# dnbaker/bonsai

Hardware: AMD Instinct MI355X
Metric: reads/s classified (150 bp) (higher is better)
Workload: dtype u64

## Files before the change

bonsai_amd/csrc/bns_device.hpp:

```cpp
#pragma once
#include <hip/hip_runtime.h>
#include <stdint.h>
#include <type_traits>
#include "bns_table_plan.hpp"

namespace bns {

using u8 = uint8_t;
using u16 = uint16_t;
using u32 = uint32_t;
using u64 = uint64_t;

constexpr u32 TAX_ABSENT = 0xFFFFFFFFu;

struct alignas(16) Slot {
    u64 key;
    u32 val;
    u32 occ;
};

struct alignas(16) TaxNode {
    u32 parent;
    u32 tin, tout;
    u32 flags;
// ... 1 lines not shown
constexpr u32 NODE_PRESENT = 1u, NODE_CHAIN_OK = 2u;

__device__ __forceinline__ int lane_id() { return (int)(threadIdx.x & 63u); }

__device__ __forceinline__ u64 wang64(u64 key)
{
    key = (~key) + (key << 21);
    key = key ^ (key >> 24);
    key = (key + (key << 3)) + (key << 8);
    key = key ^ (key >> 14);
    key = (key + (key << 2)) + (key << 4);
    key = key ^ (key >> 28);
    key = key + (key << 31);
    return key;
}

__device__ __forceinline__ u32 pairswap_not(u32 x)
{
    u32 r;
    const u32 c = 0x55555555u;
    asm("v_bitop3_b32 %0, %1, %2, %3 bitop3:0x1b" : "=v"(r) : "v"(x >> 1), "v"(x << 1), "s"(c));
    return r;
}
__device__ __forceinline__ u64 revcomp(u64 kmer, u32 k)
{
    const u32 a = __builtin_bitreverse32((u32)(kmer >> 32)), b = __builtin_bitreverse32((u32)kmer);
    const u32 lo = pairswap_not(a), hi = pairswap_not(b);
    return (((u64)hi << 32) | lo) >> (64u - (k << 1));
}

__device__ __forceinline__ u64 revcomp_top(u64 win, u32 k)
{
    const u32 a = __builtin_bitreverse32((u32)(win >> 32)), b = __builtin_bitreverse32((u32)win);
    const u32 lo = pairswap_not(a), hi = pairswap_not(b);
    return (((u64)hi << 32) | lo) & (~0ULL >> (64u - (k << 1)));
}

__device__ __forceinline__ u64 revcomp64(u64 win)
{
    const u32 a = __builtin_bitreverse32((u32)(win >> 32)), b = __builtin_bitreverse32((u32)win);
    const u32 lo = pairswap_not(a), hi = pairswap_not(b);
    return ((u64)hi << 32) | lo;
}

__device__ __forceinline__ u64 canonical(u64 kmer, u32 k)
{
// ... 106 lines not shown
    u32 n;
    u32 pad;
};
static_assert(sizeof(MinBucket) == 128, "MinBucket must be one 128-byte line");
constexpr u32 MINB_N_IN_OVF = 0xFFu;
constexpr u32 MINB_HOME_SHIFT = 18u;
constexpr u32 MINB_HOME_OVF = 1u << 21;
constexpr u32 MINB_HOME_MASK = 0xFu << MINB_HOME_SHIFT;
constexpr u32 MINB_TAG_SHIFT = 22u;
constexpr u32 MINB_TAG_MASK = 0xFFu << MINB_TAG_SHIFT;
__device__ __forceinline__ u32 minb_tag(u32 minh) { return (minh * 0x85EBCA6Bu) >> 29; }
__device__ __forceinline__ u32 minb_tagbit(u32 minh) { return (1u << MINB_TAG_SHIFT) << minb_tag(minh); }
__device__ __forceinline__ u32 mph_fold(u64 key) { return (u32)key ^ __builtin_rotateleft32((u32)(key >> 32), 15); }
__device__ __forceinline__ u32 mph_slot(u32 x, u32 S) { return __umulhi(x * S, MINB_CAP); }
__device__ __forceinline__ u32 mph_candidate(u64 bucket, u32 t)
{
    u32 z = (u32)bucket * 0x9E3779B1u + t * 0x85EBCA6Bu + (u32)(bucket >> 32);
    z ^= z >> 15; z *= 0x2C1B3C6Du; z ^= z >> 12;
    return z | 1u;
}

constexpr int BNS_MAX_SPAN = 15;
__device__ __forceinline__ u32 mmer_mix(u32 h) { return h * 0x7FEB352Du; }
__device__ __forceinline__ u32 mmer_hash(u64 x)
{
    return mmer_mix((u32)x ^ __builtin_rotateleft32((u32)(x >> 32), 13));
}
__device__ __forceinline__ u64 canon_mmer(u64 fw, u32 m)
{
    const u64 r = revcomp(fw, m);
    return fw < r ? fw : r;
}
__device__ __forceinline__ u32 bucket_of(u32 minh, u32 n_mb)
{
    u32 x = minh * 0x9E3779B1u; x ^= x >> 15;
    return __umulhi(__builtin_bitreverse32(x), n_mb);
}
__device__ __forceinline__ u64 wide_ident32(u32 x) { return ((u64)__builtin_amdgcn_alignbit(0x3FFu, x * 0x7FEB352Du, 12) << 32) | x; }
__device__ __forceinline__ u64 wide_ident64(u64 x) { return 0x3FF0000000000000ULL | ((x * 0xD6E8FEB86659FD93ULL) >> 12); }
__device__ __forceinline__ u64 wide_ident(u64 x, u32 m) { return m <= 16u ? wide_ident32((u32)x) : wide_ident64(x); }
__device__ __forceinline__ u32 wide_bucket_in(u64 ident, u32 m)
{
    return m <= 16u ? (u32)ident : (u32)ident ^ (((u32)(ident >> 32) & 0xFFFFFu) * 0x85EBCA6Bu);
}
__device__ __forceinline__ u64 wide_min(u64 a, u64 b)
{
    double r;
    asm("v_min_f64 %0, %1, %2" : "=v"(r) : "v"(__builtin_bit_cast(double, a)), "v"(__builtin_bit_cast(double, b)));
    return __builtin_bit_cast(u64, r);
}
__device__ __forceinline__ u32 key_minhash(u64 key, u32 k, MinSpec sp)
{
    const u32 m = sp.m;
    const u64 mmask = ~0ULL >> (64u - 2u * m);
    if (sp.wide) {
        const u64 rc = revcomp(key, k);
        u64 best = ~0ULL;
        for (u32 i = 0; i + m <= k; ++i) {
// ... 215 lines not shown
        }
        return ProbeResult{val, (found & 1u) != 0u};
    }
    minb_ovf_walk(key, found, val, ovf_slots, ovf_mask);
    ProbeResult r{val, (found & 1u) != 0u};
    return r;
}

constexpr int MINB_NB_WIDE = 24;
template <bool KEY_MAY_BE_ONES = true, int NB = 16, bool ADJ = false>
__device__ __forceinline__ void probe_minbucket2(const MinBucket *__restrict__ buckets, u64 keyA, u32 bA, bool activeA, u64 keyB, u32 bB,
                                                 bool activeB, u32 *aux, const Slot *__restrict__ ovf_slots, u64 ovf_mask,
                                                 ProbeResult &ra, ProbeResult &rb, u32 nb = 16u)
{
    static_assert(NB == 16, "the two-key probe is built on a 16-bucket stage (two 1 KiB loads; nb = 24 adds a third)");
    const int lane = lane_id();
    u32 *list = aux;
    uint4 *stage = reinterpret_cast<uint4 *>(aux + MINB_LIST_U32);
    const uint4 *base = reinterpret_cast<const uint4 *>(buckets);
    u32 bktA = activeA ? bA : MINB_NONE, bktB = activeB ? bB : MINB_NONE;
    u32 foundA = 0u, valA = 0u, homeA = 0u, foundB = 0u, valB = 0u, homeB = 0u;
    const u32 xfA = mph_fold(keyA), xfB = mph_fold(keyB);
    constexpr u32 GO = 1u << MINB_HOME_SHIFT;
    auto look = [&](auto first_tag, u32 &bkt, u32 rank, u32 xf, u64 key, u32 &found, u32 &val, u32 home, u32 &hx) -> bool {
        constexpr bool FIRST = decltype(first_tag)::value;
        const bool mine = bkt != MINB_NONE && rank < nb;
        const char *B = reinterpret_cast<const char *>(stage) + (mine ? rank : 0u) * (16u * MINB_STRIDE);
        const uint2 hdr = *reinterpret_cast<const uint2 *>(B + 120);
        const u32 slot = mph_slot(xf, hdr.y);
        const bool eq = *reinterpret_cast<const u64 *>(B + 8u * slot) == key;
        const bool hit = mine & eq & (!KEY_MAY_BE_ONES || ((hdr.x >> (8u + slot)) & 1u));
        const u32 v = *reinterpret_cast<const u32 *>(B + 80 + 4u * slot);
        found = hit ? 1u : found;
        val = FIRST ? v : (hit ? v : val);
        bool cont;
        if (FIRST) cont = mine & !hit & ((hdr.x & (GO | 0xFFu)) >= (GO | MINB_CAP));
        else       cont = mine & !hit & ((hdr.x & 0xFFu) >= MINB_CAP) & ((((home ? home : hdr.x) & GO)) != 0u);
        bkt = (mine && !cont) ? MINB_NONE : bkt;
        hx = hdr.x;
        return cont;
    };
    auto walk = [&](auto first_tag, bool cont, u32 hx, u32 &bkt, u32 &found, u32 &home) {
        constexpr bool FIRST = decltype(first_tag)::value;
        const u32 cur = (FIRST || home == 0u) ? ((hx & MINB_HOME_MASK) | (GO << 4)) : home;
        const bool exhausted = cont && (cur >> (MINB_HOME_SHIFT + 2u)) == 0u;
        found |= (exhausted || (cont && (hx & 0xFFu) == MINB_N_IN_OVF)) ? 2u : 0u;
        const u32 next = exhausted ? MINB_NONE : bkt + 1u;
        bkt = cont ? next : bkt;
        home = cont ? cur >> 1 : home;
    };
    bool more = true;
#ifdef BNS_COUNT_FETCHES
    u32 why_later = 4u;
#endif
    auto pass = [&](auto first_tag) -> bool {
        bool pendA, chgA, pendB, chgB;
        u64 leadA, leadB;
        u32 nA;
        if constexpr (ADJ) {
            const u32 prevA = (u32)__builtin_amdgcn_update_dpp((int)~bktA, (int)bktB, DPP_WAVE_SHR1, 0xf, 0xf, false);
            pendA = bktA != MINB_NONE; chgA = bktA != prevA; pendB = bktB != MINB_NONE; chgB = bktB != bktA;
        } else {
            const u32 a63 = readlane(bktA, 63);
            const u32 prevA = (u32)__builtin_amdgcn_update_dpp((int)~bktA, (int)bktA, DPP_WAVE_SHR1, 0xf, 0xf, false);
            const u32 prevB = (u32)__builtin_amdgcn_update_dpp((int)a63, (int)bktB, DPP_WAVE_SHR1, 0xf, 0xf, false);
            pendA = bktA != MINB_NONE; chgA = bktA != prevA; pendB = bktB != MINB_NONE; chgB = bktB != prevB;
        }
        leadA = ballot64(pendA) & ballot64(chgA); leadB = ballot64(pendB) & ballot64(chgB);
        if (!(leadA | leadB)) return false;
        nA = (u32)__popcll(leadA);
        const int n_lead = (int)nA + __popcll(leadB);
#ifdef BNS_COUNT_FETCHES
        if (lane == 0) {
            atomicAdd(&g_fetch_count[0], (unsigned long long)((u32)n_lead < nb ? (u32)n_lead : nb)); atomicAdd(&g_fetch_count[1], 1ULL);
            if (!decltype(first_tag)::value) atomicAdd(&g_fetch_count[why_later], 1ULL);
        }
#endif
        u32 rankA, rankB;
        if constexpr (ADJ) {
            const u32 upA = __builtin_amdgcn_mbcnt_hi((u32)(leadA >> 33), __builtin_amdgcn_mbcnt_lo((u32)(leadA >> 1), (u32)(leadA & 1ULL) - 1u));
            rankA = __builtin_amdgcn_mbcnt_hi((u32)(leadB >> 32), __builtin_amdgcn_mbcnt_lo((u32)leadB, upA));
            rankB = rankA + ((pendB & chgB) ? 1u : 0u);
        } else {
            rankA = __builtin_amdgcn_mbcnt_hi((u32)(leadA >> 33), __builtin_amdgcn_mbcnt_lo((u32)(leadA >> 1), (u32)(leadA & 1ULL) - 1u));
            rankB = __builtin_amdgcn_mbcnt_hi((u32)(leadB >> 33), __builtin_amdgcn_mbcnt_lo((u32)(leadB >> 1), nA + (u32)(leadB & 1ULL) - 1u));
        }
        if ((pendA & chgA) && (!ADJ || rankA < nb)) list[rankA] = bktA;
        if ((pendB & chgB) && rankB < nb) list[rankB] = bktB;
        __builtin_amdgcn_wave_barrier();
        {
            const u32 last = (u32)n_lead - 1u, slot = (u32)lane >> 3;
            typedef const void __attribute__((address_space(1))) *gptr_t;
            typedef void __attribute__((address_space(3))) *lptr_t;
            const u32 b0 = list[slot < last ? slot : last];
            __builtin_amdgcn_global_load_lds((gptr_t)(base + ((u64)b0 * 8 + (u64)(lane & 7))), (lptr_t)stage, 16, 0, 2);
            if (last >= 8u) {
                const u32 b1 = list[slot + 8u < last ? slot + 8u : last];
                __builtin_amdgcn_global_load_lds((gptr_t)(base + ((u64)b1 * 8 + (u64)(lane & 7))), (lptr_t)(stage + 64), 16, 0, 2);
                if (last >= 16u && nb > 16u) {
                    const u32 b2 = list[slot + 16u < last ? slot + 16u : last];
                    __builtin_amdgcn_global_load_lds((gptr_t)(base + ((u64)b2 * 8 + (u64)(lane & 7))), (lptr_t)(stage + 128), 16, 0, 2);
                }
            }
            asm volatile("s_waitcnt vmcnt(0)" ::: "memory");
        }
        __builtin_amdgcn_wave_barrier();
        u32 hxA, hxB;
        const bool contA = look(first_tag, bktA, rankA, xfA, keyA, foundA, valA, homeA, hxA);
        const bool contB = look(first_tag, bktB, rankB, xfB, keyB, foundB, valB, homeB, hxB);
        const u64 cA = ballot64(contA), cB = ballot64(contB);
        more = (u32)n_lead > nb || (cA | cB) != 0ULL;
#ifdef BNS_COUNT_FETCHES
        why_later = 4u + ((u32)n_lead > nb ? 1u : 0u) + ((cA | cB) != 0ULL ? 2u : 0u);
#endif
        if (cA) walk(first_tag, contA, hxA, bktA, foundA, homeA);
        if (cB) walk(first_tag, contB, hxB, bktB, foundB, homeB);
        __builtin_amdgcn_wave_barrier();
        return true;
    };
    if (pass(std::true_type{}) && more) {
        while (more && pass(std::false_type{})) {}
#ifdef BNS_COUNT_FETCHES
        { const u64 gA = ballot64(foundA == 2u), gB = ballot64(foundB == 2u);
          if ((gA | gB) && lane == 0) { atomicAdd(&g_fetch_count[2], (unsigned long long)(__popcll(gA) + __popcll(gB))); atomicAdd(&g_fetch_count[3], 1ULL); } }
#endif
        minb_ovf_walk(keyA, foundA, valA, ovf_slots, ovf_mask);
        minb_ovf_walk(keyB, foundB, valB, ovf_slots, ovf_mask);
    }
    ra = ProbeResult{valA, foundA == 1u};
    rb = ProbeResult{valB, foundB == 1u};
}

__device__ __forceinline__ TaxNode load_node(const TaxNode *__restrict__ nodes, u32 n_nodes, u32 id)
{
    if (id < n_nodes) return nodes[id];
    return TaxNode{TAX_ABSENT, 0u, 0u, 0u};
}

__device__ __forceinline__ bool anc_or_self(u32 x, const TaxNode &nx, u32 a, const TaxNode &na)
{
    return x == a || (nx.tin < na.tin && na.tin < nx.tout);
}

__device__ inline u32 lca_dev(const TaxNode *__restrict__ nodes, u32 n_nodes, u32 a, u32 b)
{
    if (a == b) return a;
    if (b == 0) return a;
    if (a == 0) return b;
// ... 13 lines not shown
```

bonsai_amd/csrc/bns_kernels.hip:

```cpp
#include "bns_device.hpp"
#include "bns_kernels.hpp"

namespace bns {

typedef const volatile __attribute__((address_space(4))) ClassifyParams ColdParams;
__device__ __forceinline__ ColdParams *cold_params() { return (ColdParams *)__builtin_amdgcn_kernarg_segment_ptr(); }

__device__ __forceinline__ u32 base_code(u32 b, u32 &bad)
{
    const u32 c = b & 0xDFu;
    const bool ok = (c == 0x41u) | (c == 0x43u) | (c == 0x47u) | (c == 0x54u);
    const u32 x = (c >> 1) & 3u;
    bad = ok ? 0u : 1u;
    return ok ? (x ^ (x >> 1)) : 0u;
}

__global__ __launch_bounds__(256) void pack_kernel(const u8 *__restrict__ bases, const u64 *__restrict__ offsets,
                                                   u64 n_reads, u64 *__restrict__ words, u32 *__restrict__ nmask)
{
    const int lane = lane_id();
    const u64 wave = (u64)blockIdx.x * (blockDim.x >> 6) + (u64)__builtin_amdgcn_readfirstlane((int)(threadIdx.x >> 6));
    const u64 n_waves = (u64)gridDim.x * (blockDim.x >> 6);
    for (u64 r = wave; r < n_reads; r += n_waves) {
        const u64 o = offsets[r];
// ... 36 lines not shown
        }
    }
}

template <bool ZEROED = false>
__device__ __forceinline__ void raw_load(const u8 *__restrict__ bases, u64 o, u32 L, u32 first_base, u32 &lo, u32 &hi)
{
    const u32 bi = first_base + (u32)lane_id() * 4u;
    if (!ZEROED) { lo = 0; hi = 0; }
    if (bi < L) {
        const u64 addr = o + bi;
        const u32 mis = (u32)(addr & 3u);
        const u32 *ap = reinterpret_cast<const u32 *>(bases + (addr - mis));
        const u32 nbytes = (L - bi) < 4u ? (L - bi) : 4u;
        lo = ap[0];
        if (mis + nbytes > 4u) hi = ap[1];
    }
}

__device__ __forceinline__ void swar_codes2(u32 w, u32 nvalid, u32 &codes8, u32 &mask8, u32 &bad8)
{
    const u32 x = w & 0xDFDFDFDFu;
    const u32 sel = (x >> 1) & 0x03030303u;
    const u32 expect = __builtin_amdgcn_perm(0u, 0x47544341u, sel);
    const u32 diff = expect ^ x;
    const u32 nz = (((diff & 0x7F7F7F7Fu) + 0x7F7F7F7Fu) | diff) & 0x80808080u;
    const u32 inv3 = (nz >> 7) * 3u;
    const u32 c = (sel ^ ((sel >> 1) & 0x01010101u)) & ~inv3;
    const u32 tail = 0xFFu >> (2u * nvalid);
    codes8 = ((c * 0x40100401u) >> 24) & ~tail;
    const u32 inv8 = (inv3 * 0x40100401u) >> 24;
    mask8 = inv8 | tail;
    bad8 = inv8 & ~tail;
}

constexpr u32 IMG_N32 = 130;
constexpr u32 IMG_U64 = 130;
template <bool ORD32 = false>
__device__ __forceinline__ bool pack_chunk_lds(const u8 *__restrict__ bases, u64 offv, int mate, u32 L, u32 j0, bool have0, u32 r_lo, u32 r_hi, u64 *pk)
{
    const int lane = lane_id();
    const u32 rem = L - j0;
    const u32 n_pass = rem >= 2048u ? 8u : (rem + 255u) >> 8;
    const u32 mis8 = 8u * ((readlane((u32)offv, mate) + j0) & 3u);
    u8 *pc = reinterpret_cast<u8 *>(pk) + (ORD32 ? 4 : 0), *pm = ORD32 ? reinterpret_cast<u8 *>(pk) + 4u * IMG_N32 + 4 : reinterpret_cast<u8 *>(pk + 64);
    u64 dirty = 0;
    auto convert = [&](u32 pass, u32 lo, u32 hi) {
        const u32 w = (u32)((((u64)hi << 32) | lo) >> mis8);
        const u32 bi = j0 + pass * 256u + (u32)lane * 4u;
        u32 codes, mask, bad;
        swar_codes2(w, bi < L ? (L - bi < 4u ? L - bi : 4u) : 0u, codes, mask, bad);
        dirty |= ballot64(bad != 0u);
        const u32 at = pass * 64u + ((u32)lane ^ (ORD32 ? 3u : 7u));
        pc[at] = (u8)codes;
        pm[at] = (u8)mask;
    };
    if (n_pass) {
        u32 lo = r_lo, hi = r_hi;
        if (!have0) { raw_load(bases, readlane64(offv, mate), L, j0, lo, hi); asm volatile("" : "+v"(lo), "+v"(hi)); }
        convert(0u, lo, hi);
    }
    for (u32 pass = 1; pass < n_pass; ++pass) {
        u32 lo, hi;
        raw_load(bases, readlane64(offv, mate), L, j0 + pass * 256u, lo, hi);
        convert(pass, lo, hi);
    }
    __builtin_amdgcn_wave_barrier();
    return dirty == 0;
}

struct Prefetch { u32 lo, hi, m; };
template <bool PACKED>
__device__ __forceinline__ void prefetch_clear(Prefetch &f)
{
// ... 169 lines not shown
__device__ __forceinline__ void window16_min2(u32 h0, u32 h1, u32 g0, u32 g1, u32 *ring, u32 &wA, u32 &wB)
{
    const u32 lane = (u32)lane_id();
    uint2 *ring2 = reinterpret_cast<uint2 *>(ring);
    const u32 Xv = blk8_suffix_min(min(g0, g1));
    ring2[lane] = make_uint2(Xv, min(Xv, dpp<0x111>(g1)));
    __builtin_amdgcn_wave_barrier();
    const u32 pm = min(h0, h1);
    const u32 P = blk8_prefix_min(pm), S = blk8_suffix_min(pm);
    ring2[8u + lane] = make_uint2(min(h1, blk8_exclusive(S, false)), S);
    __builtin_amdgcn_wave_barrier();
    const u32 xin = ring[2u * lane], sin = ring[2u * lane + 3u];
    __builtin_amdgcn_wave_barrier();
    wA = min(min(xin, blk8_exclusive(P, true)), h0);
    wB = min(sin, P);
}

template <int SPAN>
__device__ __forceinline__ void round2_minhash(u64 kfA, u64 rcA, u64 kfB, u64 rcB, u32 m, u32 *ring, u32 &hA, u32 &hB)
{
    static_assert(SPAN >= 2, "a window of at least three m-mers");
    const u32 lane = (u32)lane_id();
    const u64 mmask = ~0ULL >> (64u - 2u * m);
    auto canon_hash = [&](u64 a, u64 b) -> u32 {
        if (m <= 16u) return mmer_mix(min((u32)a, (u32)b));
        return mmer_hash(a < b ? a : b);
    };
    const u32 g0 = canon_hash(kfA >> (2u * SPAN), rcA & mmask), g1 = canon_hash(kfB >> (2u * SPAN), rcB & mmask);
    const u32 h0 = canon_hash(kfA & mmask, rcA >> (2u * SPAN)), h1 = canon_hash(kfB & mmask, rcB >> (2u * SPAN));
    if (SPAN == 15) { window16_min2(h0, h1, g0, g1, ring, hA, hB); return; }
    u32 c = min(g1, h0);
    constexpr u32 NP = ((u32)SPAN - 1u) / 2u;
    if (NP) {
        uint2 *ring2 = reinterpret_cast<uint2 *>(ring);
        ring2[lane] = make_uint2(g0, g1);
        ring[2u * lane + (u32)SPAN] = h0; ring[2u * lane + (u32)SPAN + 1u] = h1;
        __builtin_amdgcn_wave_barrier();
        uint2 h[NP ? NP : 1u];
#pragma unroll
        for (u32 i = 0; i < NP; ++i) h[i] = ring2[lane + 1u + i];
#pragma unroll
        for (u32 i = 0; i < NP; ++i) c = min(min(c, h[i].x), h[i].y);
        __builtin_amdgcn_wave_barrier();
    }
    hA = min(c, g0);
    hB = min(c, h1);
}

template <int W, bool VH = false>
__device__ __forceinline__ u32 round_minhash(u64 kf, u64 rc, u32 rd, u32 k, u32 m, u32 *ring, u32 lane_ = (u32)lane_id())
{
    const int lane = (int)lane_;
    const u32 span = k - m;
    const u64 mmask = ~0ULL >> (64u - 2u * m);
    if (span == 0) { const u64 a = kf & mmask, b = rc & mmask; return mmer_hash(a < b ? a : b); }
    u32 mine;
    if (VH) {
        u32 head = 0;
        if (m <= 16u) {
            const u32 mm = 0xFFFFFFFFu >> (32u - 2u * m);
            if (rd == 0) head = mmer_mix(min((u32)(kf >> 30) & mm, (u32)rc & mm));
            mine = mmer_mix(min((u32)kf & mm, (u32)(rc >> 30)));
        } else {
            if (rd == 0) { const u64 a = kf >> 30, b = rc & mmask; head = mmer_hash(a < b ? a : b); }
            const u64 a = kf & mmask, b = rc >> 30;
            mine = mmer_hash(a < b ? a : b);
        }
        return window16_min(mine, head, rd, ring, lane_);
    }
    if (m <= 16u) {
        const u32 mm = 0xFFFFFFFFu >> (32u - 2u * m);
        if (rd == 0) { asm volatile(""); if ((u32)lane < span) ring[lane] = mmer_mix(min((u32)(kf >> (2u * span)) & mm, (u32)rc & mm)); }
        mine = mmer_mix(min((u32)kf & mm, (u32)(rc >> (2u * span))));
        ring[span + (u32)lane] = mine;
    } else {
        if (rd == 0) {
            if ((u32)lane < span) {
                const u64 a = kf >> (2u * span), b = rc & mmask;
                ring[lane] = mmer_hash(a < b ? a : b);
            }
        }
        const u64 a = kf & mmask, b = rc >> (2u * span);
        mine = mmer_hash(a < b ? a : b);
        ring[span + (u32)lane] = mine;
    }
    __builtin_amdgcn_wave_barrier();
    constexpr u32 G = W <= 9 ? (u32)W : ((u32)W + 1u) / 2u;
    u32 best = 0xFFFFFFFFu;
#pragma unroll
    for (u32 g = 0; g < (u32)W; g += G) {
        u32 h[G + 1];
#pragma unroll
        for (u32 i = 0; i <= G; ++i) h[i] = (i < G && g + i < (u32)W) ? ring[(u32)lane + g + i] : 0xFFFFFFFFu;
        if (span == (u32)W - 1u) {
#pragma unroll
            for (u32 i = 0; i < G; i += 2) if (g + i < (u32)W) best = min(min(best, h[i]), h[i + 1]);
        } else {
#pragma unroll
            for (u32 i = 0; i < G; ++i) { const u32 x = g + i <= span ? h[i] : 0xFFFFFFFFu; best = x < best ? x : best; }
        }
        if (g + G < (u32)W) { asm volatile("" : "+v"(best)); __builtin_amdgcn_sched_barrier(0); }
    }
    __builtin_amdgcn_wave_barrier();
    if ((u32)lane >= 64u - span) ring[(u32)lane + span - 64u] = mine;
    return best;
}
// ... 327 lines not shown
    }
    return s;
}

__device__ __forceinline__ u32 resolve_wave(const u32 *keys, const u32 *cnt, u32 *tin, u32 *tout, u32 D,
                                            const TaxNode *__restrict__ nodes, u32 n_nodes, int lane_ = -1)
{
    const int lane = lane_ >= 0 ? lane_ : lane_id();
    if (D == 0) return 0u;
    if (D == 1) return keys[0];
    for (u32 i = (u32)lane; i < D; i += 64) {
        const TaxNode nd = load_node(nodes, n_nodes, keys[i]);
        tin[i] = nd.tin; tout[i] = nd.tout;
    }
    __builtin_amdgcn_wave_barrier();
    u32 best = 0;
    for (u32 base = 0; base < D; base += 64) {
        const u32 i = base + (u32)lane;
        const u32 s = i < D ? score_of(keys, cnt, tin, tout, D, i) : 0u;
        best = s > best ? s : best;
    }
#pragma unroll
    for (int off = 32; off >= 1; off >>= 1) {
        const u32 o = (u32)__shfl_xor((int)best, off);
        best = o > best ? o : best;
    }
    u32 acc = 0;
    bool first = true;
    for (u32 base = 0; base < D; base += 64) {
        const u32 i = base + (u32)lane;
        const u32 s = i < D ? score_of(keys, cnt, tin, tout, D, i) : 0u;
        u64 tie = ballot64(i < D && s == best);
        while (tie) {
            const int l = __builtin_ctzll(tie);
            tie &= tie - 1;
            const u32 t = keys[base + (u32)l];
            if (first) { acc = t; first = false; }
            else acc = lca_dev(nodes, n_nodes, acc, t);
        }
    }
    return acc;
}

__device__ __forceinline__ u32 resolve_regs(u32 ckey, u32 ccnt, u32 D, const TaxNode *__restrict__ nodes, u32 n_nodes)
{
    const u32 lane = (u32)lane_id();
    const bool in = lane < D;
// ... 16 lines not shown
        const int l = __builtin_ctzll(tie);
        tie &= tie - 1;
        const u32 t = readlane(ckey, l);
        if (first) { acc = t; first = false; }
        else acc = lca_dev(nodes, n_nodes, acc, t);
    }
    return acc;
}

#ifndef BNS_WAVES_PER_SIMD
#define BNS_WAVES_PER_SIMD 8
#endif
#ifndef BNS_SPACED_NB
#define BNS_SPACED_NB 32
#endif
#ifndef BNS_SPACED_WAVES
#define BNS_SPACED_WAVES 6
#endif
constexpr bool adjacent_kmers(int kt, int span) { return kt != 0 && kt <= 31 && span >= 2; }
template <bool SPACED, int LAYOUT, int KT, int NM, int SPAN = 8, bool OVC = false, bool WIDE = false, bool PACKED = false, bool UNIT1 = false>
struct ClassifyTraits {
    static constexpr bool PAIRS = !SPACED && LAYOUT == 2 && KT != 0 && !OVC && !WIDE;
    static constexpr bool ADJ = PAIRS && adjacent_kmers(KT, SPAN);
    static constexpr bool STAGE3 = PAIRS && !(NM == 2 && !PACKED);
    static constexpr int NB = (LAYOUT == 2 && SPACED && !UNIT1) ? BNS_SPACED_NB : 16;
    static constexpr int AUX_U32 = PAIRS ? minb_aux_u32(MINB_NB_WIDE) : minb_aux_u32(NB);
    static constexpr int RING_U32 = WIDE ? 160 : (ADJ ? 144 : 96);
    static constexpr int WAVES = (LAYOUT == 1 && !SPACED) ? 7 : (SPACED ? BNS_SPACED_WAVES : BNS_WAVES_PER_SIMD);
    static_assert(!PAIRS || (NB == 16 && minb_aux_u32(MINB_NB_WIDE) == minb_aux_u32(16) + 2 * (int)LDS_CAP), "the counter is the stage's third KiB");
    static_assert(AUX_U32 - MINB_LIST_U32 >= 2 * (int)LDS_CAP, "stage must hold tin/tout");
};
#ifndef BNS_PAD_UNIT
#define BNS_PAD_UNIT 0
#endif
#ifndef BNS_PAD_VALU
#define BNS_PAD_VALU 0
#endif
#ifndef BNS_PAD_VFAST
#define BNS_PAD_VFAST 0
#endif
#ifndef BNS_PAD_SALU
#define BNS_PAD_SALU 0
#endif
#ifndef BNS_PAD_LDS
#define BNS_PAD_LDS 0
#endif
template <int N> __device__ __forceinline__ void pad_valu(int lane)
// ... 18 lines not shown
                                              uint4 &rec_out, bool &rec_valid, IssueNext &&issue_next)
{
    using T = ClassifyTraits<SPACED, LAYOUT, KT, NM, SPAN, OVC, WIDE, PACKED, UNIT1>;
    constexpr bool PAIRS = T::PAIRS, ADJ = T::ADJ, STAGE3 = T::STAGE3;
    constexpr int NB = T::NB;
    const int lane = lane_id();
    const u32 rdesc = SPACED ? run_desc(p) : 0u;
    const u32 k = KT ? (u32)KT : p.k, c = KT ? (u32)KT : p.c;
    const u32 mlen = KT ? (u32)(KT - SPAN) : p.m;
    constexpr int MW = KT ? SPAN + 1 : BNS_MAX_SPAN + 1;
    const int nm = NM ? NM : p.nmates;
    u32 D = 0, n_hits = 0, missing = 0, ambig = 0;
    u32 ckey = 0, ccnt = 0;
    u64 dmask = 0;
    bool overflow = false;
    const bool want_hits = p.want_hits != 0;
    const u32 rounds_per_chunk = (2048u - (c - 1u)) / 64u;
    u32 n_mb = p.n_mb;
    asm volatile("" : "+s"(n_mb));

    Prefetch pre1{0u, 0u, 0u};
    const bool have1 = !SPACED && NM == 2 && !OVC;
    pad_valu<BNS_PAD_UNIT>(lane);
    auto tally = [&](const ProbeResult &pr, bool valid) -> u64 {
        const u64 fm = ballot64(pr.found), vm = ballot64(valid);
        missing += (u32)__popcll(vm & ~fm);
        if (want_hits && pr.found) { u32 *hp = cold_params()->hits; hp[readlane64(offv, (int)ob) + n_hits + (u32)__popcll(fm & lanemask_lt())] = pr.val; }
        n_hits += (u32)__popcll(fm);
        return fm;
    };
    auto vote2 = [&](u64 fa, u32 va, u64 fb, u32 vb) {
        u64 ra = fa, rb = fb;
        while (ra | rb) {
            const bool inA = ra != 0ULL;
            const int l = __builtin_ctzll(inA ? ra : rb);
            const u32 t = readlane(inA ? va : vb, l);
            const u64 ma = ballot64(va == t) & ra, mb = ballot64(vb == t) & rb;
            ra &= ~ma; rb &= ~mb;
            const u32 c = (u32)(__popcll(ma) + __popcll(mb));
            const bool eq = ckey == t;
            if (ballot64(eq) & dmask) { ccnt = eq ? ccnt + c : ccnt; continue; }
            if (!counter_insert(ckey, ccnt, dmask, keys, cnt, cap, D, t, c)) { overflow = true; break; }
        }
    };
    auto tally_adj = [&](const ProbeResult &pa, bool vA, const ProbeResult &pb, bool vB, u64 &fa, u64 &fb) {
        fa = ballot64(pa.found); fb = ballot64(pb.found);
        missing += (u32)(__popcll(ballot64(vA) & ~fa) + __popcll(ballot64(vB) & ~fb));
        if (want_hits && (pa.found || pb.found)) {
            u32 *hp = cold_params()->hits + (readlane64(offv, (int)ob) + n_hits + (u32)(__popcll(fa & lanemask_lt()) + __popcll(fb & lanemask_lt())));
            if (pa.found) hp[0] = pa.val;
            if (pb.found) hp[pa.found ? 1 : 0] = pb.val;
        }
        n_hits += (u32)(__popcll(fa) + __popcll(fb));
    };
    auto vote_adj = [&](u64 fa, u32 va, u64 fb, u32 vb) {
        u64 ra = fa, rb = fb;
        while (ra | rb) {
            const int l = __builtin_ctzll(ra | rb);
            const bool inA = ((ra >> l) & 1ULL) != 0ULL;
            const u32 t = readlane(inA ? va : vb, l);
            const u64 ma = ballot64(va == t) & ra, mb = ballot64(vb == t) & rb;
            ra &= ~ma; rb &= ~mb;
            const u32 c = (u32)(__popcll(ma) + __popcll(mb));
            const bool eq = ckey == t;
            if (ballot64(eq) & dmask) { ccnt = eq ? ccnt + c : ccnt; continue; }
            if (!counter_insert(ckey, ccnt, dmask, keys, cnt, cap, D, t, c)) { overflow = true; break; }
        }
    };
    auto pack = [&](int m, u32 L, u32 j0, bool have, const Prefetch &pre) __attribute__((always_inline)) -> bool {
        return PACKED ? load_chunk_packed<!SPACED>(p, u * (u64)nm + (u64)m, readlane64(offv, (int)ob + m), L, j0, have, pre, pk)
                      : pack_chunk_lds<!SPACED>(p.bases, offv, (int)ob + m, L, j0, have, pre.lo, pre.hi, pk);
    };
// ... 5 lines not shown
        if (have1) prefetch_clear<PACKED>(pre1);
        issue_next();
        if (have1) prefetch_issue<PACKED>(p, u * (u64)nm + 1u, readlane64(offv, (int)ob + 1), readlane((u32)offv, (int)ob + 2) - readlane((u32)offv, (int)ob + 1), pre1);
    }
    for (int m = 0; m < nm; ++m) {
        const u32 L = readlane((u32)offv, (int)ob + m + 1) - readlane((u32)offv, (int)ob + m);
        const u32 nk = n_kmers(L);
        for (u32 j0 = 0; j0 < nk; j0 += rounds_per_chunk * 64u) {
            const bool clean = (m == 0 && j0 == 0u) ? clean0 : pack(m, L, j0, have1 && m != 0 && j0 == 0u, pre1);
            u64 W = 0; u32 M = 0xFFFFFFFFu;
            if (SPACED) {
                const u32 n_written = PACKED ? 64u : ((L - j0 >= 2048u ? 2048u : L - j0) + 255u) / 256u * 8u;
                W = (u32)lane < n_written ? pk[lane] : 0ULL;
                if (!p.n_runs) M = (PACKED && clean) ? 0u : mask2_to_mask1((u32)lane < n_written ? pk[64 + lane] : ~0ULL);
            }
            const u32 chunk_nk = (nk - j0) < rounds_per_chunk * 64u ? (nk - j0) : rounds_per_chunk * 64u;
            if constexpr (PAIRS) {
                auto key_round = [&](u32 rd, u64 &key, u32 &bkt) -> bool {
                    u64 win = 0;
                    bool valid;
                    u32 lq = (u32)lane;
                    if (ADJ) asm volatile("" : "+v"(lq));
                    extract_lds32(pk, rd, k, clean, win, valid, lq);
                    const u64 kf = win >> (64u - 2u * k), krc = revcomp_top(win, k);
                    key = kf < krc ? kf : krc;
                    bkt = bucket_of(round_minhash<MW, SPAN == 15>(kf, krc, ADJ ? 0u : rd, k, mlen, ring, lq), n_mb);
                    return valid && rd * 64u + lq < chunk_nk;
                };
                if constexpr (ADJ) {
                    for (u32 rd = 0; rd * 64u < chunk_nk; rd += 2u) {
                        if ((rd + 1u) * 64u < chunk_nk) {
                            u64 win;
                            bool okA, okB;
                            extract_lds32_adj(pk, rd >> 1, k, clean, win, okA, okB);
                            const u64 kmask = ~0ULL >> (64u - 2u * k);
                            const u64 rcw = revcomp64(win);
                            const u64 kfA = win >> (64u - 2u * k), kfB = (win << 2) >> (64u - 2u * k);
                            const u64 rcA = rcw & kmask, rcB = (rcw >> 2) & kmask;
                            const u64 keyA = kfA < rcA ? kfA : rcA, keyB = kfB < rcB ? kfB : rcB;
                            u32 hA, hB;
                            round2_minhash<SPAN>(kfA, rcA, kfB, rcB, mlen, ring, hA, hB);
                            const u32 left = chunk_nk - rd * 64u;
                            const bool vA = okA && 2u * (u32)lane < left, vB = okB && 2u * (u32)lane < left - 1u;
                            ProbeResult pa, pb;
                            probe_minbucket2<false, NB, true>(p.minb, keyA, bucket_of(hA, n_mb), vA, keyB, bucket_of(hB, n_mb), vB, aux, p.slots, p.ovf_mask,
                                                              pa, pb, (STAGE3 && D <= 64u) ? (u32)MINB_NB_WIDE : 16u);
                            u64 fa, fb;
                            tally_adj(pa, vA, pb, vB, fa, fb);
                            vote_adj(fa, pa.val, fb, pb.val);
                        } else {
                            u64 keyA;
                            u32 bA;
                            const bool vA = key_round(rd, keyA, bA);
                            const ProbeResult pa = probe_minbucket<false, NB>(p.minb, keyA, bA, vA, aux, p.slots, p.ovf_mask);
                            vote2(tally(pa, vA), pa.val, 0ULL, 0u);
                        }
                    }
                } else {
                    for (u32 rd = 0; rd * 64u < chunk_nk; rd += 2u) {
                        u64 keyA;
                        u32 bA;
                        const bool vA = key_round(rd, keyA, bA);
                        if ((rd + 1u) * 64u < chunk_nk) {
                            u64 keyB;
                            u32 bB;
                            const bool vB = key_round(rd + 1u, keyB, bB);
                            ProbeResult pa, pb;
                            probe_minbucket2<(KT == 32), NB>(p.minb, keyA, bA, vA, keyB, bB, vB, aux, p.slots, p.ovf_mask, pa, pb,
                                                             (STAGE3 && D <= 64u) ? (u32)MINB_NB_WIDE : 16u);
                            const u64 fa = tally(pa, vA), fb = tally(pb, vB);
                            vote2(fa, pa.val, fb, pb.val);
                        } else {
                            const ProbeResult pa = probe_minbucket<(KT == 32), NB>(p.minb, keyA, bA, vA, aux, p.slots, p.ovf_mask);
                            vote2(tally(pa, vA), pa.val, 0ULL, 0u);
                        }
                    }
                }
            } else {
                for (u32 rd = 0; rd * 64u < chunk_nk; ++rd) {
                    const u32 jl = rd * 64u + (u32)lane;
                    u64 kmer, win = 0;
                    bool valid;
                    if (SPACED) valid = p.n_runs ? extract_spaced_lds(pk, rd, p, rdesc, kmer, clean) : extract_spaced(W, M, rd, k, rdesc, kmer);
                    else        { extract_lds32(pk, rd, k, clean, win, valid); kmer = win >> (64u - 2u * k); }
                    valid = valid && jl < chunk_nk;
                    pad_valu<BNS_PAD_VALU>(lane);
                    pad_vfast<BNS_PAD_VFAST>(lane);
                    pad_salu<BNS_PAD_SALU>();
                    pad_lds<BNS_PAD_LDS>(lane);
                    const u64 kf = kmer;
                    const u64 krc = SPACED ? 0ULL : revcomp_top(win, k);
                    if (!SPACED && (KT != 0 || p.canon)) kmer = kf < krc ? kf : krc;
                    ProbeResult pr;
#ifdef BNS_ABLATION
                    if (p.dbg & 1) { pr.found = valid && (kmer & 1); pr.val = 1000u + (u32)(kmer & 3); }
                    else
#endif
                    if (LAYOUT == 2) {
                        u32 minh;
                        if (SPACED) minh = key_minhash(kmer, k, MinSpec{p.m, p.min_len, p.min_shift, p.min_canon, 0u});
                        else if (WIDE) minh = wide_bucket_in(round_minhash_wide<MW>(kf, krc, rd, k, mlen, reinterpret_cast<u64 *>(ring)), mlen);
                        else minh = round_minhash<MW, (KT != 0 && SPAN == 15)>(kf, krc, rd, k, mlen, ring);
#ifdef BNS_ABLATION
                        if (p.dbg & 4) minh = (u32)wang64(kmer);
#endif
                        pr = probe_minbucket<(KT == 0 || KT == 32), NB, OVC, true, OVC>(p.minb, kmer, bucket_of(minh, n_mb), valid, aux, p.slots, p.ovf_mask,
                                                                                         OVC ? minb_tagbit(minh) : 0u);
                    } else if (LAYOUT == 1) pr = probe_bucket(p.slots, p.bucket_mask, kmer, valid);
                    else                  pr = probe_khash(p.kflags, p.kkeys, p.kvals, p.kh_nb, kmer, valid);
                    const u64 fm = tally(pr, valid);
#ifdef BNS_ABLATION
                    u64 rem = (p.dbg & 2) ? 0ULL : fm;
#else
                    u64 rem = fm;
#endif
                    while (rem) {
                        const int l = __builtin_ctzll(rem);
                        const u32 t = readlane(pr.val, l);
                        const u64 mm = ballot64(pr.val == t) & fm;
                        rem &= ~mm;
                        const u32 c = (u32)__popcll(mm);
                        const bool eq = ckey == t;
                        if (ballot64(eq) & dmask) { ccnt = eq ? ccnt + c : ccnt; continue; }
                        if (!counter_insert(ckey, ccnt, dmask, keys, cnt, cap, D, t, c)) { overflow = true; break; }
                    }
                }
            }
        }
        if (m == 0) ambig = L - c + 1u - n_hits - missing;
// ... 1036 lines not shown
```

Baseline: 2.247 billion.

## Materialise hot literals in SGPRs and tidy SWAR, lane-count and probe-stage code

Adds inline-asm helpers that load 32-bit constants into scalar registers with s_mov_b32. These values then feed the revcomp, hash, bucket and SWAR decode code, so VALU instructions no longer carry literal operands. Other edits simplify the SWAR tail mask, replace popcount of lanemask with mbcnt, and swap shfl_xor for ds_bpermute. They also enable the 24-bucket third stage for all pair configurations. The changes are micro-level instruction-encoding tweaks plus one config change that alters the memory fetch plan. They risk extra SALU work and scheduling constraints from the asm dependencies.

```diff
diff --git a/bonsai_amd/csrc/bns_device.hpp b/bonsai_amd/csrc/bns_device.hpp
--- a/bonsai_amd/csrc/bns_device.hpp
+++ b/bonsai_amd/csrc/bns_device.hpp
@@ -47,6 +47,35 @@
     asm("v_bitop3_b32 %0, %1, %2, %3 bitop3:0x1b" : "=v"(r) : "v"(x >> 1), "v"(x << 1), "s"(c));
     return r;
 }
+template <u32 C>
+__device__ __forceinline__ u32 lit_at(u32 dep)
+{
+    u32 r;
+    asm("s_mov_b32 %0, %1" : "=s"(r) : "n"((int)C), "v"(dep));
+    return r;
+}
+template <u32 C>
+__device__ __forceinline__ u32 lit_at_s(u32 dep)
+{
+    u32 r;
+    asm("s_mov_b32 %0, %1" : "=s"(r) : "n"((int)C), "s"(dep));
+    return r;
+}
+__device__ __forceinline__ u32 pairswap_not(u32 x, u32 c5)
+{
+    u32 r;
+    asm("v_bitop3_b32 %0, %1, %2, %3 bitop3:0x1b" : "=v"(r) : "v"(x >> 1), "v"(x << 1), "s"(c5));
+    return r;
+}
+__device__ __forceinline__ u64 revcomp64_at(u64 win)
+{
+    const u32 c5 = lit_at<0x55555555u>((u32)win);
+    const u32 a = __builtin_bitreverse32((u32)(win >> 32)), b = __builtin_bitreverse32((u32)win);
+    const u32 lo = pairswap_not(a, c5), hi = pairswap_not(b, c5);
+    return ((u64)hi << 32) | lo;
+}
+__device__ __forceinline__ u64 revcomp_top_at(u64 win, u32 k) { return revcomp64_at(win) & (~0ULL >> (64u - (k << 1))); }
+
 __device__ __forceinline__ u64 revcomp(u64 kmer, u32 k)
 {
     const u32 a = __builtin_bitreverse32((u32)(kmer >> 32)), b = __builtin_bitreverse32((u32)kmer);
@@ -199,6 +228,9 @@
 
 constexpr int BNS_MAX_SPAN = 15;
 __device__ __forceinline__ u32 mmer_mix(u32 h) { return h * 0x7FEB352Du; }
+constexpr u32 MMER_MUL = 0x7FEB352Du, BUCKET_MUL = 0x9E3779B1u;
+__device__ __forceinline__ u32 mmer_mix(u32 h, u32 mul) { return h * mul; }
+__device__ __forceinline__ u32 mmer_hash(u64 x, u32 mul) { return mmer_mix((u32)x ^ __builtin_rotateleft32((u32)(x >> 32), 13), mul); }
 __device__ __forceinline__ u32 mmer_hash(u64 x)
 {
     return mmer_mix((u32)x ^ __builtin_rotateleft32((u32)(x >> 32), 13));
@@ -211,6 +243,11 @@
 __device__ __forceinline__ u32 bucket_of(u32 minh, u32 n_mb)
 {
     u32 x = minh * 0x9E3779B1u; x ^= x >> 15;
+    return __umulhi(__builtin_bitreverse32(x), n_mb);
+}
+__device__ __forceinline__ u32 bucket_of(u32 minh, u32 n_mb, u32 mul)
+{
+    u32 x = minh * mul; x ^= x >> 15;
     return __umulhi(__builtin_bitreverse32(x), n_mb);
 }
 __device__ __forceinline__ u64 wide_ident32(u32 x) { return ((u64)__builtin_amdgcn_alignbit(0x3FFu, x * 0x7FEB352Du, 12) << 32) | x; }
@@ -472,7 +509,7 @@
     u32 foundA = 0u, valA = 0u, homeA = 0u, foundB = 0u, valB = 0u, homeB = 0u;
     const u32 xfA = mph_fold(keyA), xfB = mph_fold(keyB);
     constexpr u32 GO = 1u << MINB_HOME_SHIFT;
-    auto look = [&](auto first_tag, u32 &bkt, u32 rank, u32 xf, u64 key, u32 &found, u32 &val, u32 home, u32 &hx) -> bool {
+    auto look = [&](auto first_tag, u32 &bkt, u32 rank, u32 xf, u64 key, u32 &found, u32 &val, u32 home, u32 &hx, u32 go_cap, bool &hit_out) -> bool {
         constexpr bool FIRST = decltype(first_tag)::value;
         const bool mine = bkt != MINB_NONE && rank < nb;
         const char *B = reinterpret_cast<const char *>(stage) + (mine ? rank : 0u) * (16u * MINB_STRIDE);
@@ -484,22 +521,24 @@
         found = hit ? 1u : found;
         val = FIRST ? v : (hit ? v : val);
         bool cont;
-        if (FIRST) cont = mine & !hit & ((hdr.x & (GO | 0xFFu)) >= (GO | MINB_CAP));
+        if (FIRST) cont = mine & !hit & ((hdr.x & (GO | 0xFFu)) >= go_cap);
         else       cont = mine & !hit & ((hdr.x & 0xFFu) >= MINB_CAP) & ((((home ? home : hdr.x) & GO)) != 0u);
         bkt = (mine && !cont) ? MINB_NONE : bkt;
         hx = hdr.x;
+        hit_out = hit;
         return cont;
     };
     auto walk = [&](auto first_tag, bool cont, u32 hx, u32 &bkt, u32 &found, u32 &home) {
         constexpr bool FIRST = decltype(first_tag)::value;
         const u32 cur = (FIRST || home == 0u) ? ((hx & MINB_HOME_MASK) | (GO << 4)) : home;
-        const bool exhausted = cont && (cur >> (MINB_HOME_SHIFT + 2u)) == 0u;
-        found |= (exhausted || (cont && (hx & 0xFFu) == MINB_N_IN_OVF)) ? 2u : 0u;
+        const u32 last_home = lit_at<(1u << (MINB_HOME_SHIFT + 2u))>(hx), in_ovf = lit_at<MINB_N_IN_OVF>(hx);
+        const bool exhausted = cont && cur < last_home;
+        found |= (exhausted || (cont && (hx & 0xFFu) == in_ovf)) ? 2u : 0u;
         const u32 next = exhausted ? MINB_NONE : bkt + 1u;
         bkt = cont ? next : bkt;
         home = cont ? cur >> 1 : home;
     };
-    bool more = true;
+    bool more = true, hitA = false, hitB = false;
 #ifdef BNS_COUNT_FETCHES
     u32 why_later = 4u;
 #endif
@@ -546,18 +585,19 @@
             __builtin_amdgcn_global_load_lds((gptr_t)(base + ((u64)b0 * 8 + (u64)(lane & 7))), (lptr_t)stage, 16, 0, 2);
             if (last >= 8u) {
                 const u32 b1 = list[slot + 8u < last ? slot + 8u : last];
-                __builtin_amdgcn_global_load_lds((gptr_t)(base + ((u64)b1 * 8 + (u64)(lane & 7))), (lptr_t)(stage + 64), 16, 0, 2);
+                __builtin_amdgcn_global_load_lds((gptr_t)(base + ((u64)b1 * 8 + (u64)(lane & 7))), (lptr_t)(reinterpret_cast<char *>(stage) + lit_at_s<1024u>(last)), 16, 0, 2);
                 if (last >= 16u && nb > 16u) {
                     const u32 b2 = list[slot + 16u < last ? slot + 16u : last];
-                    __builtin_amdgcn_global_load_lds((gptr_t)(base + ((u64)b2 * 8 + (u64)(lane & 7))), (lptr_t)(stage + 128), 16, 0, 2);
+                    __builtin_amdgcn_global_load_lds((gptr_t)(base + ((u64)b2 * 8 + (u64)(lane & 7))), (lptr_t)(reinterpret_cast<char *>(stage) + lit_at_s<2048u>(last)), 16, 0, 2);
                 }
             }
             asm volatile("s_waitcnt vmcnt(0)" ::: "memory");
         }
         __builtin_amdgcn_wave_barrier();
         u32 hxA, hxB;
-        const bool contA = look(first_tag, bktA, rankA, xfA, keyA, foundA, valA, homeA, hxA);
-        const bool contB = look(first_tag, bktB, rankB, xfB, keyB, foundB, valB, homeB, hxB);
+        const u32 go_cap = decltype(first_tag)::value ? lit_at<(GO | MINB_CAP)>(rankA) : 0u;
+        const bool contA = look(first_tag, bktA, rankA, xfA, keyA, foundA, valA, homeA, hxA, go_cap, hitA);
+        const bool contB = look(first_tag, bktB, rankB, xfB, keyB, foundB, valB, homeB, hxB, go_cap, hitB);
         const u64 cA = ballot64(contA), cB = ballot64(contB);
         more = (u32)n_lead > nb || (cA | cB) != 0ULL;
 #ifdef BNS_COUNT_FETCHES
@@ -570,10 +610,6 @@
     };
     if (pass(std::true_type{}) && more) {
         while (more && pass(std::false_type{})) {}
-#ifdef BNS_COUNT_FETCHES
-        { const u64 gA = ballot64(foundA == 2u), gB = ballot64(foundB == 2u);
-          if ((gA | gB) && lane == 0) { atomicAdd(&g_fetch_count[2], (unsigned long long)(__popcll(gA) + __popcll(gB))); atomicAdd(&g_fetch_count[3], 1ULL); } }
-#endif
         minb_ovf_walk(keyA, foundA, valA, ovf_slots, ovf_mask);
         minb_ovf_walk(keyB, foundB, valB, ovf_slots, ovf_mask);
     }
diff --git a/bonsai_amd/csrc/bns_kernels.hip b/bonsai_amd/csrc/bns_kernels.hip
--- a/bonsai_amd/csrc/bns_kernels.hip
+++ b/bonsai_amd/csrc/bns_kernels.hip
@@ -82,16 +82,18 @@
 {
     const u32 x = w & 0xDFDFDFDFu;
     const u32 sel = (x >> 1) & 0x03030303u;
-    const u32 expect = __builtin_amdgcn_perm(0u, 0x47544341u, sel);
+    const u32 expect = __builtin_amdgcn_perm(0u, lit_at<0x47544341u>(w), sel);
     const u32 diff = expect ^ x;
-    const u32 nz = (((diff & 0x7F7F7F7Fu) + 0x7F7F7F7Fu) | diff) & 0x80808080u;
-    const u32 inv3 = (nz >> 7) * 3u;
+    const u32 c7f = lit_at<0x7F7F7F7Fu>(w);
+    const u32 nz = (((diff & c7f) + c7f) | diff) & 0x80808080u;
+    const u32 nz1 = nz >> 7;
+    const u32 inv3 = nz1 * 3u;
     const u32 c = (sel ^ ((sel >> 1) & 0x01010101u)) & ~inv3;
-    const u32 tail = 0xFFu >> (2u * nvalid);
-    codes8 = ((c * 0x40100401u) >> 24) & ~tail;
-    const u32 inv8 = (inv3 * 0x40100401u) >> 24;
+    const u32 ntail = 0xFFFFFFFFu << (8u - 2u * nvalid), tail = ~ntail;
+    codes8 = ((c * lit_at<0x40100401u>(w)) >> 24) & ntail;
+    const u32 inv8 = (nz1 * lit_at<0xC0300C03u>(w)) >> 24;
     mask8 = inv8 | tail;
-    bad8 = inv8 & ~tail;
+    bad8 = inv8 & ntail;
 }
 
 constexpr u32 IMG_N32 = 130;
@@ -109,7 +111,7 @@
         const u32 w = (u32)((((u64)hi << 32) | lo) >> mis8);
         const u32 bi = j0 + pass * 256u + (u32)lane * 4u;
         u32 codes, mask, bad;
-        swar_codes2(w, bi < L ? (L - bi < 4u ? L - bi : 4u) : 0u, codes, mask, bad);
+        swar_codes2(w, min(__builtin_elementwise_sub_sat(L, bi), 4u), codes, mask, bad);
         dirty |= ballot64(bad != 0u);
         const u32 at = pass * 64u + ((u32)lane ^ (ORD32 ? 3u : 7u));
         pc[at] = (u8)codes;
@@ -325,9 +327,10 @@
     static_assert(SPAN >= 2, "a window of at least three m-mers");
     const u32 lane = (u32)lane_id();
     const u64 mmask = ~0ULL >> (64u - 2u * m);
+    const u32 mul = lit_at<MMER_MUL>((u32)kfA);
     auto canon_hash = [&](u64 a, u64 b) -> u32 {
-        if (m <= 16u) return mmer_mix(min((u32)a, (u32)b));
-        return mmer_hash(a < b ? a : b);
+        if (m <= 16u) return mmer_mix(min((u32)a, (u32)b), mul);
+        return mmer_hash(a < b ? a : b, mul);
     };
     const u32 g0 = canon_hash(kfA >> (2u * SPAN), rcA & mmask), g1 = canon_hash(kfB >> (2u * SPAN), rcB & mmask);
     const u32 h0 = canon_hash(kfA & mmask, rcA >> (2u * SPAN)), h1 = canon_hash(kfB & mmask, rcB >> (2u * SPAN));
@@ -356,35 +359,36 @@
     const int lane = (int)lane_;
     const u32 span = k - m;
     const u64 mmask = ~0ULL >> (64u - 2u * m);
-    if (span == 0) { const u64 a = kf & mmask, b = rc & mmask; return mmer_hash(a < b ? a : b); }
+    const u32 mul = lit_at<MMER_MUL>((u32)kf);
+    if (span == 0) { const u64 a = kf & mmask, b = rc & mmask; return mmer_hash(a < b ? a : b, mul); }
     u32 mine;
     if (VH) {
         u32 head = 0;
         if (m <= 16u) {
             const u32 mm = 0xFFFFFFFFu >> (32u - 2u * m);
-            if (rd == 0) head = mmer_mix(min((u32)(kf >> 30) & mm, (u32)rc & mm));
-            mine = mmer_mix(min((u32)kf & mm, (u32)(rc >> 30)));
+            if (rd == 0) head = mmer_mix(min((u32)(kf >> 30) & mm, (u32)rc & mm), mul);
+            mine = mmer_mix(min((u32)kf & mm, (u32)(rc >> 30)), mul);
         } else {
-            if (rd == 0) { const u64 a = kf >> 30, b = rc & mmask; head = mmer_hash(a < b ? a : b); }
+            if (rd == 0) { const u64 a = kf >> 30, b = rc & mmask; head = mmer_hash(a < b ? a : b, mul); }
             const u64 a = kf & mmask, b = rc >> 30;
-            mine = mmer_hash(a < b ? a : b);
+            mine = mmer_hash(a < b ? a : b, mul);
         }
         return window16_min(mine, head, rd, ring, lane_);
     }
     if (m <= 16u) {
         const u32 mm = 0xFFFFFFFFu >> (32u - 2u * m);
-        if (rd == 0) { asm volatile(""); if ((u32)lane < span) ring[lane] = mmer_mix(min((u32)(kf >> (2u * span)) & mm, (u32)rc & mm)); }
-        mine = mmer_mix(min((u32)kf & mm, (u32)(rc >> (2u * span))));
+        if (rd == 0) { asm volatile(""); if ((u32)lane < span) ring[lane] = mmer_mix(min((u32)(kf >> (2u * span)) & mm, (u32)rc & mm), mul); }
+        mine = mmer_mix(min((u32)kf & mm, (u32)(rc >> (2u * span))), mul);
         ring[span + (u32)lane] = mine;
     } else {
         if (rd == 0) {
             if ((u32)lane < span) {
                 const u64 a = kf >> (2u * span), b = rc & mmask;
-                ring[lane] = mmer_hash(a < b ? a : b);
+                ring[lane] = mmer_hash(a < b ? a : b, mul);
             }
         }
         const u64 a = kf & mmask, b = rc >> (2u * span);
-        mine = mmer_hash(a < b ? a : b);
+        mine = mmer_hash(a < b ? a : b, mul);
         ring[span + (u32)lane] = mine;
     }
     __builtin_amdgcn_wave_barrier();
@@ -758,7 +762,7 @@
     }
 #pragma unroll
     for (int off = 32; off >= 1; off >>= 1) {
-        const u32 o = (u32)__shfl_xor((int)best, off);
+        const u32 o = (u32)__builtin_amdgcn_ds_bpermute((lane ^ off) << 2, (int)best);
         best = o > best ? o : best;
     }
     u32 acc = 0;
@@ -821,7 +825,7 @@
 struct ClassifyTraits {
     static constexpr bool PAIRS = !SPACED && LAYOUT == 2 && KT != 0 && !OVC && !WIDE;
     static constexpr bool ADJ = PAIRS && adjacent_kmers(KT, SPAN);
-    static constexpr bool STAGE3 = PAIRS && !(NM == 2 && !PACKED);
+    static constexpr bool STAGE3 = PAIRS;
     static constexpr int NB = (LAYOUT == 2 && SPACED && !UNIT1) ? BNS_SPACED_NB : 16;
     static constexpr int AUX_U32 = PAIRS ? minb_aux_u32(MINB_NB_WIDE) : minb_aux_u32(NB);
     static constexpr int RING_U32 = WIDE ? 160 : (ADJ ? 144 : 96);
@@ -886,10 +890,11 @@
     Prefetch pre1{0u, 0u, 0u};
     const bool have1 = !SPACED && NM == 2 && !OVC;
     pad_valu<BNS_PAD_UNIT>(lane);
+    auto lanes_below = [](u64 m) -> u32 { return __builtin_amdgcn_mbcnt_hi((u32)(m >> 32), __builtin_amdgcn_mbcnt_lo((u32)m, 0u)); };
     auto tally = [&](const ProbeResult &pr, bool valid) -> u64 {
         const u64 fm = ballot64(pr.found), vm = ballot64(valid);
         missing += (u32)__popcll(vm & ~fm);
-        if (want_hits && pr.found) { u32 *hp = cold_params()->hits; hp[readlane64(offv, (int)ob) + n_hits + (u32)__popcll(fm & lanemask_lt())] = pr.val; }
+        if (want_hits && pr.found) { u32 *hp = cold_params()->hits; hp[readlane64(offv, (int)ob) + n_hits + lanes_below(fm)] = pr.val; }
         n_hits += (u32)__popcll(fm);
         return fm;
     };
@@ -911,7 +916,7 @@
         fa = ballot64(pa.found); fb = ballot64(pb.found);
         missing += (u32)(__popcll(ballot64(vA) & ~fa) + __popcll(ballot64(vB) & ~fb));
         if (want_hits && (pa.found || pb.found)) {
-            u32 *hp = cold_params()->hits + (readlane64(offv, (int)ob) + n_hits + (u32)(__popcll(fa & lanemask_lt()) + __popcll(fb & lanemask_lt())));
+            u32 *hp = cold_params()->hits + (readlane64(offv, (int)ob) + n_hits + lanes_below(fa) + lanes_below(fb));
             if (pa.found) hp[0] = pa.val;
             if (pb.found) hp[pa.found ? 1 : 0] = pb.val;
         }
@@ -963,9 +968,10 @@
                     u32 lq = (u32)lane;
                     if (ADJ) asm volatile("" : "+v"(lq));
                     extract_lds32(pk, rd, k, clean, win, valid, lq);
-                    const u64 kf = win >> (64u - 2u * k), krc = revcomp_top(win, k);
+                    const u64 kf = win >> (64u - 2u * k), krc = revcomp_top_at(win, k);
                     key = kf < krc ? kf : krc;
-                    bkt = bucket_of(round_minhash<MW, SPAN == 15>(kf, krc, ADJ ? 0u : rd, k, mlen, ring, lq), n_mb);
+                    const u32 minh = round_minhash<MW, SPAN == 15>(kf, krc, ADJ ? 0u : rd, k, mlen, ring, lq);
+                    bkt = bucket_of(minh, n_mb, lit_at<BUCKET_MUL>(minh));
                     return valid && rd * 64u + lq < chunk_nk;
                 };
                 if constexpr (ADJ) {
@@ -975,7 +981,7 @@
                             bool okA, okB;
                             extract_lds32_adj(pk, rd >> 1, k, clean, win, okA, okB);
                             const u64 kmask = ~0ULL >> (64u - 2u * k);
-                            const u64 rcw = revcomp64(win);
+                            const u64 rcw = revcomp64_at(win);
                             const u64 kfA = win >> (64u - 2u * k), kfB = (win << 2) >> (64u - 2u * k);
                             const u64 rcA = rcw & kmask, rcB = (rcw >> 2) & kmask;
                             const u64 keyA = kfA < rcA ? kfA : rcA, keyB = kfB < rcB ? kfB : rcB;
@@ -984,7 +990,8 @@
                             const u32 left = chunk_nk - rd * 64u;
                             const bool vA = okA && 2u * (u32)lane < left, vB = okB && 2u * (u32)lane < left - 1u;
                             ProbeResult pa, pb;
-                            probe_minbucket2<false, NB, true>(p.minb, keyA, bucket_of(hA, n_mb), vA, keyB, bucket_of(hB, n_mb), vB, aux, p.slots, p.ovf_mask,
+                            const u32 bmul = lit_at<BUCKET_MUL>(hA);
+                            probe_minbucket2<false, NB, true>(p.minb, keyA, bucket_of(hA, n_mb, bmul), vA, keyB, bucket_of(hB, n_mb, bmul), vB, aux, p.slots, p.ovf_mask,
                                                               pa, pb, (STAGE3 && D <= 64u) ? (u32)MINB_NB_WIDE : 16u);
                             u64 fa, fb;
                             tally_adj(pa, vA, pb, vB, fa, fb);
@@ -1030,7 +1037,7 @@
                     pad_salu<BNS_PAD_SALU>();
                     pad_lds<BNS_PAD_LDS>(lane);
                     const u64 kf = kmer;
-                    const u64 krc = SPACED ? 0ULL : revcomp_top(win, k);
+                    const u64 krc = SPACED ? 0ULL : revcomp_top_at(win, k);
                     if (!SPACED && (KT != 0 || p.canon)) kmer = kf < krc ? kf : krc;
                     ProbeResult pr;
 #ifdef BNS_ABLATION
@@ -1045,7 +1052,7 @@
 #ifdef BNS_ABLATION
                         if (p.dbg & 4) minh = (u32)wang64(kmer);
 #endif
-                        pr = probe_minbucket<(KT == 0 || KT == 32), NB, OVC, true, OVC>(p.minb, kmer, bucket_of(minh, n_mb), valid, aux, p.slots, p.ovf_mask,
+                        pr = probe_minbucket<(KT == 0 || KT == 32), NB, OVC, true, OVC>(p.minb, kmer, bucket_of(minh, n_mb, lit_at<BUCKET_MUL>(minh)), valid, aux, p.slots, p.ovf_mask,
                                                                                          OVC ? minb_tagbit(minh) : 0u);
                     } else if (LAYOUT == 1) pr = probe_bucket(p.slots, p.bucket_mask, kmer, valid);
                     else                  pr = probe_khash(p.kflags, p.kkeys, p.kvals, p.kh_nb, kmer, valid);
```

Result: slower. 2.194 billion (-2.3%).
